# Nostrademous/dotaclient

Measured on AMD Instinct MI355X. Metric: PPO optimizer samples/sec (whole node) + actor steps/sec, 1v1-mid LSTM policy, higher is better.
Workload: dtype fp32

## Files before the change

### dotaclient_amd/ops/csrc/lstm_team.hip

```cpp
#include "common.h"
#include <cstdlib>

namespace {

using dca::bf16x8;
typedef int i32x4 __attribute__((ext_vector_type(4)));
typedef unsigned u32x2 __attribute__((ext_vector_type(2)));

constexpr int kT = 32;
constexpr int kMaxTeams = 8;
constexpr int kThreads = 256;
constexpr int kSc1 = 16;
constexpr int kPlain = 0;
constexpr unsigned kSpinLimit = 1u << 22;

struct TeamCtl {
  unsigned xcnt[16];
  unsigned state[kMaxTeams];
  unsigned chain[kMaxTeams];
  unsigned done[kMaxTeams];
  unsigned next_chain;
  unsigned abort;
  unsigned exits;
  unsigned epoch;
};
static_assert(sizeof(TeamCtl) <= 256, "TeamCtl must fit the 256-byte control tensor");

__device__ __forceinline__ unsigned xcc_id() { return __builtin_amdgcn_s_getreg((3 << 11) | 20) & 0xf; }
__device__ __forceinline__ unsigned ld_acq(const unsigned* p) {
  return __hip_atomic_load((__attribute__((address_space(1))) unsigned*)p, __ATOMIC_RELAXED, __HIP_MEMORY_SCOPE_AGENT);
}
__device__ __forceinline__ void st_rel(unsigned* p, unsigned v) {
  __hip_atomic_store((__attribute__((address_space(1))) unsigned*)p, v, __ATOMIC_RELAXED, __HIP_MEMORY_SCOPE_AGENT);
}
__device__ __forceinline__ unsigned add_agent(unsigned* p, unsigned v) {
  return __hip_atomic_fetch_add(p, v, __ATOMIC_RELAXED, __HIP_MEMORY_SCOPE_AGENT);
}
template <typename T>
__device__ __forceinline__ void gstore(T* p, T v) { *(__attribute__((address_space(1))) T*)p = v; }
__device__ __forceinline__ void lds_barrier() { asm volatile("s_waitcnt lgkmcnt(0)\n\ts_barrier" ::: "memory"); }

__device__ __forceinline__ void split_frag(const float* __restrict__ p, bf16x8& hi, bf16x8& lo) {
  const float4 a = *reinterpret_cast<const float4*>(p), b = *reinterpret_cast<const float4*>(p + 4);
  const float v[8] = {a.x, a.y, a.z, a.w, b.x, b.y, b.z, b.w};
#pragma unroll
  for (int j = 0; j < 8; ++j) {
    hi[j] = dca::f2bf(v[j]);
    lo[j] = dca::f2bf(v[j] - dca::bf2f(hi[j]));
  }
}

typedef float f32x2 __attribute__((ext_vector_type(2)));
template <int KSL>
__device__ __forceinline__ void pk_dot4(const float* wq, const float* x, float& o0, float& o1, float& o2, float& o3) {
  f32x2 a01e = {0.f, 0.f}, a01o = {0.f, 0.f}, a23e = {0.f, 0.f}, a23o = {0.f, 0.f};
#pragma unroll
  for (int j = 0; j < KSL; j += 4) {
    const float4 v = *reinterpret_cast<const float4*>(x + j);
    a01e = __builtin_elementwise_fma(f32x2{wq[j], wq[KSL + j]}, f32x2{v.x, v.x}, a01e);
    a23e = __builtin_elementwise_fma(f32x2{wq[2 * KSL + j], wq[3 * KSL + j]}, f32x2{v.x, v.x}, a23e);
    a01o = __builtin_elementwise_fma(f32x2{wq[j + 1], wq[KSL + j + 1]}, f32x2{v.y, v.y}, a01o);
    a23o = __builtin_elementwise_fma(f32x2{wq[2 * KSL + j + 1], wq[3 * KSL + j + 1]}, f32x2{v.y, v.y}, a23o);
    a01e = __builtin_elementwise_fma(f32x2{wq[j + 2], wq[KSL + j + 2]}, f32x2{v.z, v.z}, a01e);
    a23e = __builtin_elementwise_fma(f32x2{wq[2 * KSL + j + 2], wq[3 * KSL + j + 2]}, f32x2{v.z, v.z}, a23e);
    a01o = __builtin_elementwise_fma(f32x2{wq[j + 3], wq[KSL + j + 3]}, f32x2{v.w, v.w}, a01o);
    a23o = __builtin_elementwise_fma(f32x2{wq[2 * KSL + j + 3], wq[3 * KSL + j + 3]}, f32x2{v.w, v.w}, a23o);
  }
  const f32x2 a01 = a01e + a01o, a23 = a23e + a23o;
  o0 = a01.x; o1 = a01.y; o2 = a23.x; o3 = a23.y;
}
__device__ __forceinline__ float row_sum16(float v) {
  v += __int_as_float(__builtin_amdgcn_mov_dpp(__float_as_int(v), 0xB1, 0xF, 0xF, false));
  v += __int_as_float(__builtin_amdgcn_mov_dpp(__float_as_int(v), 0x4E, 0xF, 0xF, false));
  v += __int_as_float(__builtin_amdgcn_mov_dpp(__float_as_int(v), 0x141, 0xF, 0xF, false));
  v += __int_as_float(__builtin_amdgcn_mov_dpp(__float_as_int(v), 0x140, 0xF, 0xF, false));
  return v;
}

template <bool PREC>
__device__ __forceinline__ float sigm(float x) { return PREC ? 1.f / (1.f + expf(-x)) : dca::sigmoidf_(x); }
template <bool PREC>
__device__ __forceinline__ float tanh_(float x) { return PREC ? tanhf(x) : dca::tanhf_(x); }

__device__ __forceinline__ float row_sum32(float v) {
  v = row_sum16(v);
  return v + __int_as_float(__builtin_amdgcn_ds_swizzle(__float_as_int(v), 0x401F));
}

__device__ __forceinline__ __amdgpu_buffer_rsrc_t uniform_rsrc(const void* p, int bytes) {
  const unsigned long long a = (unsigned long long)p;
  const unsigned lo = __builtin_amdgcn_readfirstlane((unsigned)a);
  const unsigned hi = __builtin_amdgcn_readfirstlane((unsigned)(a >> 32));
  return __builtin_amdgcn_make_buffer_rsrc((void*)(((unsigned long long)hi << 32) | lo), (short)0,
                                           __builtin_amdgcn_readfirstlane(bytes), 0x00020000);
}

__device__ __forceinline__ bool spin_fail(unsigned& spins, unsigned long long& since, TeamCtl* ctl, unsigned* err,
                                          unsigned code, int knobs) {
  asm volatile("" ::: "memory");
  ++spins;
  if ((spins & 255u) == 0) {
    if (ld_acq(&ctl->abort) != 0) return true;
    const unsigned long long limit = ((knobs >> 15) & 1) ? 6000000000ull : 200000000ull;
    const unsigned long long now = __builtin_amdgcn_s_memrealtime();
    if (since == 0) {
      since = now;
    } else if (now - since > limit) {
      st_rel(err, code);
      st_rel(&ctl->abort, 1u);
      return true;
    }
  }
  if (spins > 32 && !((knobs >> 13) & 1)) __builtin_amdgcn_s_sleep(1);
  return false;
}

__device__ int join_team(TeamCtl* ctl, unsigned* err, int* sh, unsigned* sh_epoch, bool refuse = false) {
  if (threadIdx.x == 0) {
    *sh_epoch = ld_acq(&ctl->epoch);
    int res = -1;
    const unsigned x = xcc_id();
    if (x < kMaxTeams && !refuse) {
      const unsigned r = add_agent(&ctl->xcnt[x], 1u);
      if (r < (unsigned)kT) {
        res = (int)x * 64 + (int)r;
        unsigned spins = 0;
        if (r == 0) {
          bool ok = false;
          while (true) {
            if (ld_acq(&ctl->xcnt[x]) >= (unsigned)kT) { ok = true; break; }
            if (++spins > (1u << 16)) break;
            __builtin_amdgcn_s_sleep(2);
          }
          st_rel(&ctl->state[x], ok ? 1u : 2u);
          if (!ok) res = -1;
        } else {
          unsigned s;
          while ((s = ld_acq(&ctl->state[x])) == 0) {
            if (++spins > (1u << 18)) break;
            __builtin_amdgcn_s_sleep(2);
          }
          if (s != 1) res = -1;
        }
      }
    }
    *sh = res;
  }
  __syncthreads();
  return *sh;
}

__device__ int next_chain(TeamCtl* ctl, int team, int member, unsigned iter, int nch, int* sh) {
  if (threadIdx.x == 0) {
    int res = -1;
    unsigned spins = 0;
    if (member == 0) {
      while (ld_acq(&ctl->done[team]) < (unsigned)kT * iter) {
        if (ld_acq(&ctl->abort) || ++spins > (1u << 24)) { spins = ~0u; break; }
        __builtin_amdgcn_s_sleep(1);
      }
      unsigned c = spins == ~0u ? 0xffffu : add_agent(&ctl->next_chain, 1u);
      if (c > 0xffffu) c = 0xffffu;
      st_rel(&ctl->chain[team], ((iter + 1) << 16) | c);
      res = (c < (unsigned)nch) ? (int)c : -1;
    } else {
      unsigned v;
      while (((v = ld_acq(&ctl->chain[team])) >> 16) != iter + 1) {
        if (ld_acq(&ctl->abort) || ++spins > (1u << 24)) { v = 0xffffu; break; }
        __builtin_amdgcn_s_sleep(1);
      }
      const unsigned c = v & 0xffffu;
      res = (c < (unsigned)nch) ? (int)c : -1;
    }
    *sh = res;
  }
  __syncthreads();
  return *sh;
}

__device__ void team_exit(TeamCtl* ctl, unsigned* err, int nch) {
  __syncthreads();
  if (threadIdx.x == 0) {
    const unsigned e = add_agent(&ctl->exits, 1u);
    if (e == gridDim.x - 1) {
      if (ld_acq(&ctl->next_chain) < (unsigned)nch) st_rel(err, 3u);
      for (int i = 0; i < 16; ++i) st_rel(&ctl->xcnt[i], 0u);
      for (int i = 0; i < kMaxTeams; ++i) {
        st_rel(&ctl->state[i], 0u);
        st_rel(&ctl->chain[i], 0u);
        st_rel(&ctl->done[i], 0u);
      }
      st_rel(&ctl->next_chain, 0u);
      st_rel(&ctl->abort, 0u);
      st_rel(&ctl->exits, 0u);
      st_rel(&ctl->epoch, ld_acq(&ctl->epoch) + 1u);
    }
  }
}

__device__ __forceinline__ unsigned make_tagbase(unsigned epoch, unsigned iter) {
  return ((epoch & 0x7ffu) << 21) | (((iter + 1u) & 0x1fu) << 16);
}

template <int MT, int KS, bool F32, int VAR>
__device__ __forceinline__ void lstm_team_fwd_body(
    const float* __restrict__ xp4, const void* __restrict__ whh_, const float* __restrict__ h0,
    const float* __restrict__ c0, short* __restrict__ hs, float* __restrict__ hsf, float* __restrict__ cs,
    float* __restrict__ gates4, float* __restrict__ hn, float* __restrict__ cn, unsigned long long* xg_all,
    TeamCtl* ctl, unsigned* err, int Btot, int Bc, int nch, int S, int sb, int st, unsigned long long* trace,
    int knobs, const float* __restrict__ bias4, const unsigned char* __restrict__ rst) {
  constexpr int H = 128 * KS;
  constexpr int U = H / kT;
  constexpr int NTILE = U / 4;
  constexpr int KSTEP = H / 32;
  constexpr int HP = H + 8;
  constexpr int RB = MT * 16;
  constexpr int VV = VAR & 3;
  constexpr bool PREC = (VAR & 4) != 0;
  constexpr bool V1 = VV >= 1;
  constexpr int NT = VV == 2 ? 512 : kThreads;
  constexpr int LPU = VV == 2 ? 32 : 16;
  constexpr int UPW = 64 / LPU;
  constexpr int KSL = H / LPU;
  constexpr int R = V1 ? (1 << ((VAR >> 5) & 3)) : 1;
  constexpr int NR = V1 ? R : MT;
  static_assert(!V1 || (F32 && MT == 1), "V1 is the fp32 exact VALU variant");
  static_assert(VV != 2 || H == 512, "V2 maps 8 waves x 2 units onto the 16 units of H = 512");
  __shared__ short hl[V1 ? 1 : 2][V1 ? 1 : RB][V1 ? 1 : HP];
  __shared__ short hlo[F32 && !V1 ? 2 : 1][F32 && !V1 ? RB : 1][F32 && !V1 ? HP : 1];
  constexpr int SP = KSL + 4;
  constexpr int ROWF = LPU * SP;
  __shared__ __attribute__((aligned(16))) float hf[V1 ? 2 : 1][V1 ? R * ROWF : 4];
  __shared__ int sh_int;
  __shared__ unsigned sh_epoch;

  const int tid = threadIdx.x, wv = tid >> 6, lane = tid & 63;
  const int me = join_team(ctl, err, &sh_int, &sh_epoch, (knobs >> 11) & 1);
  const unsigned epoch = sh_epoch;
  if (me < 0) return;
  const int team = me >> 6, m = me & 63;
  const int j0 = m * U;
#define TSTAMP(ev)                                                                                        \
  if (trace && lane == 0 && wv < 4 && chain == 0 && t < 64)                                                \
    trace[(((size_t)m * 4 + wv) * 64 + t) * 8 + (ev)] = __builtin_amdgcn_s_memrealtime()
  constexpr int GPR = F32 ? H : H / 2;
  unsigned long long* xg = xg_all + (size_t)team * 2 * Bc * GPR;

  if constexpr (!V1)
    for (int i = tid; i < 2 * RB * HP; i += NT) (&hl[0][0][0])[i] = 0;
  if constexpr (F32 && !V1)
    for (int i = tid; i < 2 * RB * HP; i += NT) (&hlo[0][0][0])[i] = 0;

  const bool mfma_wave = VV == 2 || wv < NTILE;
  const int col = lane & 15, kg = lane >> 4;
  bf16x8 wf[V1 ? 1 : KSTEP];
  bf16x8 wfl[F32 && !V1 ? KSTEP : 1];
  float wq[V1 ? 4 * KSL : 1];
  if (mfma_wave) {
    const int row = (col & 3) * H + j0 + 4 * wv + (col >> 2);
    if constexpr (V1) {
#pragma unroll
      for (int g = 0; g < 4; ++g) {
        const float* wr = static_cast<const float*>(whh_) + (size_t)(g * H + j0 + UPW * wv + lane / LPU) * H +
                          (lane % LPU) * KSL;
#pragma unroll
        for (int j = 0; j < KSL; j += 4) {
          const float4 v = *reinterpret_cast<const float4*>(wr + j);
          wq[g * KSL + j] = v.x; wq[g * KSL + j + 1] = v.y; wq[g * KSL + j + 2] = v.z; wq[g * KSL + j + 3] = v.w;
        }
      }
    } else if constexpr (F32) {
      const float* whh = static_cast<const float*>(whh_);
#pragma unroll
      for (int ks = 0; ks < KSTEP; ++ks) split_frag(whh + (size_t)row * H + ks * 32 + 8 * kg, wf[ks], wfl[ks]);
    } else {
      const short* whh = static_cast<const short*>(whh_);
#pragma unroll
      for (int ks = 0; ks < KSTEP; ++ks)
        wf[ks] = *reinterpret_cast<const bf16x8*>(whh + (size_t)row * H + ks * 32 + 8 * kg);
    }
  }
  const int erow = V1 ? (lane % LPU) : 4 * kg + (col & 3);
  const int eunit = j0 + (V1 ? UPW * wv + lane / LPU : 4 * wv + (col >> 2));
  const dca::f32x4 bv = (bias4 && mfma_wave) ? *reinterpret_cast<const dca::f32x4*>(bias4 + eunit * 4)
                                             : dca::f32x4{0.f, 0.f, 0.f, 0.f};

  const int slice = V1 ? lane % LPU : 0;
  unsigned spins = 0;
  unsigned long long since = 0;
  for (unsigned iter = 0;; ++iter) {
    const int chain = next_chain(ctl, team, m, iter, nch, &sh_int);
    if (chain < 0) break;
    const int b0 = chain * Bc;
    const int B = min(Bc, Btot - b0);
    const unsigned tagbase = make_tagbase(epoch, iter);
    float creg[NR], hreg[NR];
#pragma unroll
    for (int i = 0; i < NR; ++i) {
      const int b = V1 ? i : i * 16 + erow;
      creg[i] = (mfma_wave && b < B) ? c0[(size_t)(b0 + b) * H + eunit] : 0.f;
      hreg[i] = 0.f;
    }
    bool dead = false;
    for (int t = 0; t < S; ++t) {
      const int par = t & 1;
      spins = 0;
      since = 0;
      TSTAMP(0);
      dca::f32x4 xv[NR];
      int rzb[NR];
      if (mfma_wave) {
#pragma unroll
        for (int i = 0; i < NR; ++i) {
          const int b = V1 ? i : i * 16 + erow;
          const size_t tx = ((knobs >> 10) & 1) ? 0 : (size_t)t;
          xv[i] = (b < B) ? *reinterpret_cast<const dca::f32x4*>(xp4 + (((size_t)(b0 + b) * sb + tx * st) * H + eunit) * 4)
                          : dca::f32x4{0.f, 0.f, 0.f, 0.f};
          rzb[i] = 0;
          if (rst != nullptr)
            rzb[i] = rst[(size_t)(b0 + (b < B ? b : 0)) * sb + (size_t)t * st];
        }
      }
      if (t == 0) {
        for (int i = tid; i < B * H; i += NT) {
          const int b = i / H, k = i % H;
          const float v = h0[(size_t)(b0 + b) * H + k];
          if constexpr (V1) {
            hf[par][b * ROWF + (k / KSL) * SP + k % KSL] = v;
          } else {
            hl[par][b][k] = dca::f2bf(v);
            if constexpr (F32) hlo[par][b][k] = dca::f2bf(v - dca::bf2f(dca::f2bf(v)));
          }
        }
      } else {
        const unsigned tag = tagbase | (unsigned)t;
        const __amdgpu_buffer_rsrc_t rs = uniform_rsrc(xg + (size_t)((t - 1) & 1) * Bc * GPR, Bc * GPR * 8);
        constexpr int CPR = F32 ? H / 2 : H / 4;
        constexpr int NL = ((V1 ? R : RB) * CPR + NT - 1) / NT;
        i32x4 g[NL];
        bool okc[NL];
#pragma unroll
        for (int i = 0; i < NL; ++i) okc[i] = tid + NT * i >= B * CPR;
        for (int i = 0; i < (knobs & 0xff); ++i) __builtin_amdgcn_s_sleep(1);
        if ((knobs >> 9) & 1) {
          while (!okc[0]) {
            g[0] = __builtin_amdgcn_raw_buffer_load_b128(rs, tid * 16, 0, kSc1);
            okc[0] = ((unsigned)g[0].y == tag) & ((unsigned)g[0].w == tag);
            if (__all(okc[0])) break;
            if (spin_fail(spins, since, ctl, err, 1u, knobs)) { dead = true; break; }
          }
        }
        while (!dead) {
#pragma unroll
          for (int i = 0; i < NL; ++i)
            if (!okc[i]) g[i] = __builtin_amdgcn_raw_buffer_load_b128(rs, (tid + NT * i) * 16, 0, kSc1);
          bool ok = true;
#pragma unroll
          for (int i = 0; i < NL; ++i) {
            okc[i] = okc[i] || (((unsigned)g[i].y == tag) & ((unsigned)g[i].w == tag));
            ok &= okc[i];
          }
          if (__all(ok)) break;
          if (spin_fail(spins, since, ctl, err, 1u, knobs)) { dead = true; break; }
        }
#pragma unroll
        for (int i = 0; i < NL; ++i) {
          const int ci = tid + NT * i;
          if (ci < B * CPR) {
            if constexpr (V1) {
              const int b = ci / CPR, k = 2 * (ci % CPR);
              *reinterpret_cast<float2*>(&hf[par][b * ROWF + (k / KSL) * SP + k % KSL]) =
                  make_float2(__int_as_float(g[i].x), __int_as_float(g[i].z));
            } else if constexpr (F32) {
              const int b = ci / CPR, k = (ci % CPR) * 2;
              const float x = __int_as_float(g[i].x), z = __int_as_float(g[i].z);
              const short xh = dca::f2bf(x), zh = dca::f2bf(z);
              *reinterpret_cast<unsigned*>(&hl[par][b][k]) = (unsigned)(unsigned short)xh | ((unsigned)(unsigned short)zh << 16);
              *reinterpret_cast<unsigned*>(&hlo[par][b][k]) =
                  (unsigned)(unsigned short)dca::f2bf(x - dca::bf2f(xh)) |
                  ((unsigned)(unsigned short)dca::f2bf(z - dca::bf2f(zh)) << 16);
            } else {
              const int b = ci / CPR, k = (ci % CPR) * 4;
              *reinterpret_cast<u32x2*>(&hl[par][b][k]) = u32x2{(unsigned)g[i].x, (unsigned)g[i].z};
            }
          }
        }
      }
      TSTAMP(1);
      if (dead) sh_int = -2;
      lds_barrier();
      if (sh_int == -2) break;
      TSTAMP(2);
      if constexpr (V1) {
       if (mfma_wave) {
        float g[R][4];
#pragma unroll
        for (int r = 0; r < R; ++r) {
          if (r < B) {
            pk_dot4<KSL>(wq, &hf[par][r * ROWF + slice * SP], g[r][0], g[r][1], g[r][2], g[r][3]);
#pragma unroll
            for (int q = 0; q < 4; ++q) g[r][q] = LPU == 32 ? row_sum32(g[r][q]) : row_sum16(g[r][q]);
          }
        }
        float act[R][4], cr[R], hr[R], hpub = 0.f;
#pragma unroll
        for (int r = 0; r < R; ++r) {
          cr[r] = hr[r] = 0.f;
          act[r][0] = act[r][1] = act[r][2] = act[r][3] = 0.f;
          if (r < B) {
            if (rzb[r]) { g[r][0] = 0.f; g[r][1] = 0.f; g[r][2] = 0.f; g[r][3] = 0.f; }
            const float pi = g[r][0] + (xv[r][0] + bv[0]), pf = g[r][1] + (xv[r][1] + bv[1]),
                        pg = g[r][2] + (xv[r][2] + bv[2]), po = g[r][3] + (xv[r][3] + bv[3]);
            const float ig = sigm<PREC>(pi), fg = sigm<PREC>(pf), gg = tanh_<PREC>(pg), og = sigm<PREC>(po);
            const float c = fg * (rzb[r] ? 0.f : creg[r]) + ig * gg;
            const float hv = og * tanh_<PREC>(c);
            creg[r] = c; hreg[r] = hv; cr[r] = c; hr[r] = hv;
            act[r][0] = ig; act[r][1] = fg; act[r][2] = gg; act[r][3] = og;
            if (slice == r) hpub = hv;
          }
        }
        TSTAMP(3);
        if (slice < B) {
          const u32x2 gv = {(unsigned)__float_as_int(hpub), tagbase | (unsigned)(t + 1)};
          const __amdgpu_buffer_rsrc_t ws = uniform_rsrc(xg + (size_t)par * Bc * GPR, Bc * GPR * 8);
          __builtin_amdgcn_raw_buffer_store_b64(gv, ws, (slice * H + eunit) * 8, 0, kPlain);
        }
        TSTAMP(4);
        const int orow = slice >> 1;
        if (orow < B && orow < R && !((knobs >> 8) & 1)) {
          float cv = 0.f, hv = 0.f;
          dca::f32x4 av = {0.f, 0.f, 0.f, 0.f};
#pragma unroll
          for (int r = 0; r < R; ++r)
            if (orow == r) { cv = cr[r]; hv = hr[r]; av = dca::f32x4{act[r][0], act[r][1], act[r][2], act[r][3]}; }
          const size_t o = ((size_t)(b0 + orow) * sb + (size_t)t * st) * H + eunit;
          gstore((slice & 1) ? hsf + o : cs + o, (slice & 1) ? hv : cv);
          if (!(slice & 1)) *reinterpret_cast<dca::f32x4*>(gates4 + o * 4) = av;
        }
        TSTAMP(5);
       }
      } else if (mfma_wave) {
#pragma unroll
        for (int mt = 0; mt < MT; ++mt) {
          if (mt * 16 >= B) break;
          float gq0 = 0.f, gq1 = 0.f, gq2 = 0.f, gq3 = 0.f;
          {
          dca::f32x4 acc = {0.f, 0.f, 0.f, 0.f};
          if constexpr (F32) {
            dca::f32x4 a1 = {0.f, 0.f, 0.f, 0.f}, a2 = {0.f, 0.f, 0.f, 0.f};
#pragma unroll
            for (int ks = 0; ks < KSTEP; ++ks) {
              const bf16x8 a = *reinterpret_cast<const bf16x8*>(&hl[par][mt * 16 + col][ks * 32 + 8 * kg]);
              const bf16x8 al = *reinterpret_cast<const bf16x8*>(&hlo[par][mt * 16 + col][ks * 32 + 8 * kg]);
              acc = __builtin_amdgcn_mfma_f32_16x16x32_bf16(a, wf[ks], acc, 0, 0, 0);
              a1 = __builtin_amdgcn_mfma_f32_16x16x32_bf16(al, wf[ks], a1, 0, 0, 0);
              a2 = __builtin_amdgcn_mfma_f32_16x16x32_bf16(a, wfl[ks], a2, 0, 0, 0);
            }
            acc += a1 + a2;
          } else {
#pragma unroll
            for (int ks = 0; ks < KSTEP; ++ks) {
              const bf16x8 a = *reinterpret_cast<const bf16x8*>(&hl[par][mt * 16 + col][ks * 32 + 8 * kg]);
              acc = __builtin_amdgcn_mfma_f32_16x16x32_bf16(a, wf[ks], acc, 0, 0, 0);
            }
          }
          const int q0 = col & 3;
#pragma unroll
          for (int j = 0; j < 4; ++j) {
            const int sel = (q0 - j) & 3;
            const float send = sel == 0 ? acc[0] : sel == 1 ? acc[1] : sel == 2 ? acc[2] : acc[3];
            const int qs = (q0 + j) & 3;
            float got = send;
            if (j == 1) got = __int_as_float(__builtin_amdgcn_mov_dpp(__float_as_int(send), 0x39, 0xF, 0xF, false));
            if (j == 2) got = __int_as_float(__builtin_amdgcn_mov_dpp(__float_as_int(send), 0x4E, 0xF, 0xF, false));
            if (j == 3) got = __int_as_float(__builtin_amdgcn_mov_dpp(__float_as_int(send), 0x93, 0xF, 0xF, false));
            gq0 = qs == 0 ? got : gq0;
            gq1 = qs == 1 ? got : gq1;
            gq2 = qs == 2 ? got : gq2;
            gq3 = qs == 3 ? got : gq3;
          }
          }
          const int b = mt * 16 + erow;
          if (rzb[mt]) { gq0 = 0.f; gq1 = 0.f; gq2 = 0.f; gq3 = 0.f; }
          const float pi = gq0 + (xv[mt][0] + bv[0]), pf = gq1 + (xv[mt][1] + bv[1]), pg = gq2 + (xv[mt][2] + bv[2]),
                      po = gq3 + (xv[mt][3] + bv[3]);
          const float ig = sigm<PREC>(pi), fg = sigm<PREC>(pf), gg = tanh_<PREC>(pg), og = sigm<PREC>(po);
          const float c = fg * (rzb[mt] ? 0.f : creg[mt]) + ig * gg;
          const float hv = og * tanh_<PREC>(c);
          if (b < B) { creg[mt] = c; hreg[mt] = hv; }
          TSTAMP(3);
          if constexpr (F32) {
            if (b < B) {
              const u32x2 gv = {(unsigned)__float_as_int(hv), tagbase | (unsigned)(t + 1)};
              const __amdgpu_buffer_rsrc_t ws = uniform_rsrc(xg + (size_t)par * Bc * GPR, Bc * GPR * 8);
              __builtin_amdgcn_raw_buffer_store_b64(gv, ws, (b * H + eunit) * 8, 0, kPlain);
            }
          } else {
            const float hnb = __int_as_float(__builtin_amdgcn_mov_dpp(__float_as_int(hv), 0x104, 0xF, 0xF, false));
            if (b < B && ((col >> 2) & 1) == 0) {
              const unsigned pl = (unsigned)(unsigned short)dca::f2bf(hv) | ((unsigned)(unsigned short)dca::f2bf(hnb) << 16);
              const u32x2 gv = {pl, tagbase | (unsigned)(t + 1)};
              const __amdgpu_buffer_rsrc_t ws = uniform_rsrc(xg + (size_t)par * Bc * GPR, Bc * GPR * 8);
              __builtin_amdgcn_raw_buffer_store_b64(gv, ws, (b * (H / 2) + (eunit >> 1)) * 8, 0, kPlain);
            }
          }
          TSTAMP(4);
          if (b < B && !((knobs >> 8) & 1)) {
            const size_t bt = (size_t)(b0 + b) * sb + (size_t)t * st;
            if (hs) hs[bt * H + eunit] = dca::f2bf(hv);
            if (hsf) hsf[bt * H + eunit] = hv;
            cs[bt * H + eunit] = c;
            *reinterpret_cast<dca::f32x4*>(gates4 + (bt * H + eunit) * 4) = dca::f32x4{ig, fg, gg, og};
          }
          TSTAMP(5);
        }
      }
    }
#undef TSTAMP
    if (sh_int == -2) return;
    if (mfma_wave) {
#pragma unroll
      for (int i = 0; i < NR; ++i) {
        const int b = V1 ? i : i * 16 + erow;
        if (b < B && (!V1 || slice == i)) {
          hn[(size_t)(b0 + b) * H + eunit] = hreg[i];
          cn[(size_t)(b0 + b) * H + eunit] = creg[i];
        }
      }
    }
    __syncthreads();
    if (tid == 0) add_agent(&ctl->done[team], 1u);
  }
}

template <int MT, int KS, bool F32, int VAR>
__device__ __forceinline__ void lstm_team_bwd_body(
    const float* __restrict__ dhs, const float* __restrict__ gates4, const float* __restrict__ cs,
    const float* __restrict__ c0, const float* __restrict__ dhn, const float* __restrict__ dcn,
    const void* __restrict__ whh_, float* __restrict__ dgates4, float* __restrict__ dh0, float* __restrict__ dc0,
    i32x4* xg_all, TeamCtl* ctl, unsigned* err, int Btot, int Bc, int nch, int S, int sb, int st,
    unsigned long long* trace, short* __restrict__ dg16, float* __restrict__ dbpart, int knobs,
    const unsigned char* __restrict__ rst) {
  constexpr int H = 128 * KS;
  constexpr int U = H / kT;
  constexpr int VV = VAR & 3;
  constexpr bool PREC = (VAR & 4) != 0;
  constexpr bool V1 = VV >= 1;
  constexpr int NWK = VV == 2 ? 8 : 4;
  constexpr int NT = 64 * NWK;
  constexpr int KW = 4 * H / NWK;
  constexpr int KSTEP = KW / 32;
  constexpr int RB = MT * 16;
  constexpr int GP = 4 * H + 8;
  constexpr int KSL = KW / 16;
  constexpr int R = V1 ? (1 << ((VAR >> 5) & 3)) : 1;
  constexpr int NPAIR = ((V1 ? R : RB) * U + NT - 1) / NT;
  static_assert(!V1 || (F32 && MT == 1), "V1 is the fp32 exact VALU variant");
  static_assert(VV != 2 || H == 512, "V2 is the H = 512 variant");
  __shared__ short dgl[V1 ? 1 : RB][V1 ? 1 : GP];
  __shared__ short dglo[F32 && !V1 ? RB : 1][F32 && !V1 ? GP : 1];
  constexpr int SP = KSL + 4;
  constexpr int DROW = (4 * H / KSL) * SP;
  __shared__ __attribute__((aligned(16))) float dgf[V1 ? R * DROW : 4];
  constexpr int RR = V1 ? R : RB;
  __shared__ float red[V1 ? 2 : 1][NWK][RR][16 + 1];
  __shared__ float dbs[RB * U * 4];
  __shared__ int sh_int;
  __shared__ unsigned sh_epoch;
  constexpr int kRstWords = 2048;
  __shared__ unsigned rbits[kRstWords];

  const int tid = threadIdx.x, wv = tid >> 6, lane = tid & 63;
  const int me = join_team(ctl, err, &sh_int, &sh_epoch);
  const unsigned epoch = sh_epoch;
  if (me < 0) return;
  const int team = me >> 6, m = me & 63;
  const int j0 = m * U;
  const int wpr = (S + 31) >> 5;
  constexpr int CPU_ = F32 ? 2 : 1;
  i32x4* xg = xg_all + (size_t)team * 2 * Bc * H * CPU_;
#define TSTAMPB(ev)                                                                                       \
  if (trace && lane == 0 && wv < 4 && chain == 0 && k < 64)                                               \
    trace[(((size_t)m * 4 + wv) * 64 + k) * 8 + (ev)] = __builtin_amdgcn_s_memrealtime()

  if constexpr (!V1)
    for (int i = tid; i < RB * GP; i += NT) (&dgl[0][0])[i] = 0;
  if constexpr (F32 && !V1)
    for (int i = tid; i < RB * GP; i += NT) (&dglo[0][0])[i] = 0;

  const int col = lane & 15, kg = lane >> 4;
  bf16x8 wf[V1 ? 1 : KSTEP];
  bf16x8 wfl[F32 && !V1 ? KSTEP : 1];
  float wq[V1 ? 4 * KSL : 1];
  if constexpr (V1) {
#pragma unroll
    for (int uu = 0; uu < 4; ++uu) {
      const int unit = 16 * (wv / NWK) + 4 * (lane >> 4) + uu;
#pragma unroll
      for (int j = 0; j < KSL; ++j) {
        const int gc = (wv % NWK) * KW + (lane & 15) * KSL + j;
        wq[uu * KSL + j] =
            (unit < U) ? static_cast<const float*>(whh_)[(size_t)((gc & 3) * H + (gc >> 2)) * H + j0 + unit] : 0.f;
      }
    }
  }
#pragma unroll
  for (int ks = 0; ks < (V1 ? 0 : KSTEP); ++ks) {
    bf16x8 v, vl;
#pragma unroll
    for (int j = 0; j < 8; ++j) {
      const int gc = wv * KW + ks * 32 + 8 * kg + j;
      const size_t wi = (size_t)((gc & 3) * H + (gc >> 2)) * H + j0 + col;
      if constexpr (F32) {
        const float w = (col < U) ? static_cast<const float*>(whh_)[wi] : 0.f;
        v[j] = dca::f2bf(w);
        vl[j] = dca::f2bf(w - dca::bf2f(v[j]));
      } else {
        v[j] = (col < U) ? static_cast<const short*>(whh_)[wi] : (short)0;
      }
    }
    wf[ks] = v;
    if constexpr (F32 && !V1) wfl[ks] = vl;
  }

  unsigned spins = 0;
  unsigned long long since = 0;
  for (unsigned iter = 0;; ++iter) {
    const int chain = next_chain(ctl, team, m, iter, nch, &sh_int);
    if (chain < 0) break;
    const int b0 = chain * Bc;
    const int B = min(Bc, Btot - b0);
    const unsigned tagbase = make_tagbase(epoch, iter);
    const bool rl = rst != nullptr && B * wpr <= kRstWords;
    if (rl) {
      for (int w = tid; w < B * wpr; w += NT) {
        const int b = w / wpr, tb = (w - b * wpr) * 32;
        const unsigned char* fr = rst + (size_t)(b0 + b) * sb;
        unsigned v = 0;
#pragma unroll
        for (int j = 0; j < 32; ++j)
          if (tb + j < S) v |= (fr[(size_t)(tb + j) * st] != 0 ? 1u : 0u) << j;
        rbits[w] = v;
      }
      lds_barrier();
    }
    float dcarry[NPAIR];
    dca::f32x4 dsum[NPAIR];
#pragma unroll
    for (int i = 0; i < NPAIR; ++i) dsum[i] = dca::f32x4{0.f, 0.f, 0.f, 0.f};
#pragma unroll
    for (int i = 0; i < NPAIR; ++i) {
      const int pi = tid + NT * i;
      dcarry[i] = (pi < B * U && dcn) ? dcn[(size_t)(b0 + pi / U) * H + j0 + pi % U] : 0.f;
    }
    bool dead = false;
    for (int k = 0; k <= S; ++k) {
      const int t = S - 1 - k;
      spins = 0;
      since = 0;
      TSTAMPB(0);
      dca::f32x4 gv[NPAIR];
      float cv[NPAIR], cpv[NPAIR], dv[NPAIR];
      bool rcur[NPAIR], rnext[NPAIR];
      if (t >= 0) {
#pragma unroll
        for (int i = 0; i < NPAIR; ++i) {
          const int pi = tid + NT * i;
          rcur[i] = rnext[i] = false;
          if (pi < B * U) {
            const int b = pi / U, u = pi % U;
            const size_t bt = (size_t)(b0 + b) * sb + (size_t)t * st;
            gv[i] = *reinterpret_cast<const dca::f32x4*>(gates4 + (bt * H + j0 + u) * 4);
            cv[i] = cs[bt * H + j0 + u];
            cpv[i] = t > 0 ? cs[(bt - st) * H + j0 + u] : c0[(size_t)(b0 + b) * H + j0 + u];
            dv[i] = dhs[bt * H + j0 + u];
            if (rl) {
              const unsigned* rw = rbits + b * wpr;
              rcur[i] = (rw[t >> 5] >> (t & 31)) & 1u;
              rnext[i] = t + 1 < S && ((rw[(t + 1) >> 5] >> ((t + 1) & 31)) & 1u);
            } else if (rst != nullptr) {
              rcur[i] = rst[bt] != 0;
              rnext[i] = t + 1 < S && rst[bt + st] != 0;
            }
          }
        }
      }
      if (k > 0) {
        const unsigned tag = tagbase | (unsigned)(t + 2);
        const __amdgpu_buffer_rsrc_t rs = uniform_rsrc(xg + (size_t)((t + 1) & 1) * Bc * H * CPU_, Bc * H * CPU_ * 16);
        constexpr int RG = F32 ? 4 : 8;
        constexpr int NL = RG * H * CPU_ / NT;
        if constexpr (V1) {
          constexpr int CW = KW / 128;
          constexpr int NLW = R * CW;
          static_assert(KW % 128 == 0, "a wave's K part is whole rounds of 64 chunks");
          const int cw0 = (wv % NWK) * (KW / 2) + lane;
          i32x4 g[NLW];
          bool okc[NLW];
#pragma unroll
          for (int i = 0; i < NLW; ++i) okc[i] = i / CW >= B;
          while (true) {
#pragma unroll
            for (int i = 0; i < NLW; ++i)
              if (!okc[i])
                g[i] = __builtin_amdgcn_raw_buffer_load_b128(rs, ((i / CW) * H * CPU_ + cw0 + 64 * (i % CW)) * 16, 0, kSc1);
            bool ok = true;
#pragma unroll
            for (int i = 0; i < NLW; ++i) {
              okc[i] = okc[i] || (((unsigned)g[i].y == tag) & ((unsigned)g[i].w == tag));
              ok &= okc[i];
            }
            if (__all(ok)) break;
            if (spin_fail(spins, since, ctl, err, 2u, knobs)) { dead = true; break; }
          }
#pragma unroll
          for (int i = 0; i < NLW; ++i) {
            if (i / CW < B) {
              const int r = cw0 + 64 * (i % CW), gc = 4 * (r >> 1) + 2 * (r & 1);
              *reinterpret_cast<float2*>(&dgf[(i / CW) * DROW + (gc / KSL) * SP + gc % KSL]) =
                  make_float2(__int_as_float(g[i].x), __int_as_float(g[i].z));
            }
          }
        } else {
          for (int g0 = 0; g0 < B && !dead; g0 += RG) {
            const int nck = min(RG, B - g0) * H * CPU_;
            i32x4 g[NL];
            bool okc[NL];
#pragma unroll
            for (int i = 0; i < NL; ++i) okc[i] = tid + NT * i >= nck;
            while (true) {
#pragma unroll
              for (int i = 0; i < NL; ++i)
                if (!okc[i]) g[i] = __builtin_amdgcn_raw_buffer_load_b128(rs, (g0 * H * CPU_ + tid + NT * i) * 16, 0, kSc1);
              bool ok = true;
#pragma unroll
              for (int i = 0; i < NL; ++i) {
                okc[i] = okc[i] || (((unsigned)g[i].y == tag) & ((unsigned)g[i].w == tag));
                ok &= okc[i];
              }
              if (__all(ok)) break;
              if (spin_fail(spins, since, ctl, err, 2u, knobs)) { dead = true; break; }
            }
#pragma unroll
            for (int i = 0; i < NL; ++i) {
              const int ci = tid + NT * i;
              if (ci < nck) {
                if constexpr (F32) {
                  const int b = g0 + ci / (2 * H), r = ci % (2 * H), gc = 4 * (r >> 1) + 2 * (r & 1);
                  const float x = __int_as_float(g[i].x), z = __int_as_float(g[i].z);
                  const short xh = dca::f2bf(x), zh = dca::f2bf(z);
                  *reinterpret_cast<unsigned*>(&dgl[b][gc]) = (unsigned)(unsigned short)xh | ((unsigned)(unsigned short)zh << 16);
                  *reinterpret_cast<unsigned*>(&dglo[b][gc]) =
                      (unsigned)(unsigned short)dca::f2bf(x - dca::bf2f(xh)) |
                      ((unsigned)(unsigned short)dca::f2bf(z - dca::bf2f(zh)) << 16);
                } else {
                  const int b = g0 + ci / H, j = ci % H;
                  *reinterpret_cast<u32x2*>(&dgl[b][4 * j]) = u32x2{(unsigned)g[i].x, (unsigned)g[i].z};
                }
              }
            }
          }
        }
      }
      TSTAMPB(1);
      if constexpr (V1) {
        asm volatile("s_waitcnt lgkmcnt(0)" ::: "memory");
      } else {
        if (dead) sh_int = -2;
        lds_barrier();
        if (sh_int == -2) break;
        TSTAMPB(2);
      }
      const int rp = V1 ? (k & 1) : 0;
      if (V1 && k > 0) {
       if (!dead) {
        const int wk = wv % NWK;
        const int u0 = 16 * (wv / NWK) + 4 * (lane >> 4);
#pragma unroll
        for (int r = 0; r < R; ++r) {
          if (r >= B) break;
          float o0, o1, o2, o3;
          const float* x = &dgf[r * DROW + (wk * 16 + (lane & 15)) * SP];
          pk_dot4<KSL>(wq, x, o0, o1, o2, o3);
          o0 = row_sum16(o0);
          o1 = row_sum16(o1);
          o2 = row_sum16(o2);
          o3 = row_sum16(o3);
          if ((lane & 15) == 0 && u0 < U) {
            red[rp][wk][r][u0] = o0;
            red[rp][wk][r][u0 + 1] = o1;
            red[rp][wk][r][u0 + 2] = o2;
            red[rp][wk][r][u0 + 3] = o3;
          }
        }
       }
      } else if (k > 0) {
#pragma unroll
        for (int mt = 0; mt < MT; ++mt) {
          if (mt * 16 >= B) break;
          dca::f32x4 acc = {0.f, 0.f, 0.f, 0.f};
          if constexpr (F32) {
            dca::f32x4 a1 = {0.f, 0.f, 0.f, 0.f}, a2 = {0.f, 0.f, 0.f, 0.f};
#pragma unroll
            for (int ks = 0; ks < KSTEP; ++ks) {
              const bf16x8 a = *reinterpret_cast<const bf16x8*>(&dgl[mt * 16 + col][wv * KW + ks * 32 + 8 * kg]);
              const bf16x8 al = *reinterpret_cast<const bf16x8*>(&dglo[mt * 16 + col][wv * KW + ks * 32 + 8 * kg]);
              acc = __builtin_amdgcn_mfma_f32_16x16x32_bf16(a, wf[ks], acc, 0, 0, 0);
              a1 = __builtin_amdgcn_mfma_f32_16x16x32_bf16(al, wf[ks], a1, 0, 0, 0);
              a2 = __builtin_amdgcn_mfma_f32_16x16x32_bf16(a, wfl[ks], a2, 0, 0, 0);
            }
            acc += a1 + a2;
          } else {
#pragma unroll
            for (int ks = 0; ks < KSTEP; ++ks) {
              const bf16x8 a = *reinterpret_cast<const bf16x8*>(&dgl[mt * 16 + col][wv * KW + ks * 32 + 8 * kg]);
              acc = __builtin_amdgcn_mfma_f32_16x16x32_bf16(a, wf[ks], acc, 0, 0, 0);
            }
          }
#pragma unroll
          for (int r = 0; r < 4; ++r) red[0][wv][mt * 16 + kg * 4 + r][col] = acc[r];
        }
      }
      TSTAMPB(3);
      if (V1 && dead) sh_int = -2;
      lds_barrier();
      if (V1 && sh_int == -2) break;
      TSTAMPB(4);
      if (t < 0) {
        for (int i = tid; i < B * U; i += NT) {
          const int b = i / U, u = i % U;
          float acc = 0.f;
#pragma unroll
          for (int w = 0; w < NWK; ++w) acc += red[rp][w][b][u];
          dh0[(size_t)(b0 + b) * H + j0 + u] = (rst != nullptr && rst[(size_t)(b0 + b) * sb] != 0) ? 0.f : acc;
        }
        break;
      }
      const __amdgpu_buffer_rsrc_t ws = uniform_rsrc(xg + (size_t)(t & 1) * Bc * H * CPU_, Bc * H * CPU_ * 16);
      const int tg = (int)(tagbase | (unsigned)(t + 1));
#pragma unroll
      for (int i = 0; i < NPAIR; ++i) {
        const int pi = tid + NT * i;
        if (pi < B * U) {
          const int b = pi / U, u = pi % U;
          float rec = 0.f;
          if (k == 0) {
            rec = dhn ? dhn[(size_t)(b0 + b) * H + j0 + u] : 0.f;
          } else if (!rnext[i]) {
#pragma unroll
            for (int w = 0; w < NWK; ++w) rec += red[rp][w][b][u];
          }
          const float ig = gv[i][0], fg = gv[i][1], gg = gv[i][2], og = gv[i][3];
          const float dht = dv[i] + rec;
          const float tc = tanh_<PREC>(cv[i]);
          const float dc = dcarry[i] + dht * og * (1.f - tc * tc);
          const float d_i = dc * gg * ig * (1.f - ig);
          const float d_f = rcur[i] ? 0.f : dc * cpv[i] * fg * (1.f - fg);
          const float d_g = dc * ig * (1.f - gg * gg);
          const float d_o = dht * tc * og * (1.f - og);
          dcarry[i] = rcur[i] ? 0.f : dc * fg;
          const size_t bt = (size_t)(b0 + b) * sb + (size_t)t * st;
          if constexpr (F32) {
            const int o = (b * H + j0 + u) * 2 * 16;
            __builtin_amdgcn_raw_buffer_store_b128(i32x4{__float_as_int(d_i), tg, __float_as_int(d_f), tg}, ws, o, 0,
                                                   kPlain);
            __builtin_amdgcn_raw_buffer_store_b128(i32x4{__float_as_int(d_g), tg, __float_as_int(d_o), tg}, ws, o + 16,
                                                   0, kPlain);
            *reinterpret_cast<dca::f32x4*>(dgates4 + (bt * H + j0 + u) * 4) = dca::f32x4{d_i, d_f, d_g, d_o};
          } else {
            const unsigned p01 = (unsigned)(unsigned short)dca::f2bf(d_i) | ((unsigned)(unsigned short)dca::f2bf(d_f) << 16);
            const unsigned p23 = (unsigned)(unsigned short)dca::f2bf(d_g) | ((unsigned)(unsigned short)dca::f2bf(d_o) << 16);
            __builtin_amdgcn_raw_buffer_store_b128(i32x4{(int)p01, tg, (int)p23, tg}, ws, (b * H + j0 + u) * 16, 0, kPlain);
            if (dg16) *reinterpret_cast<u32x2*>(dg16 + (bt * H + j0 + u) * 4) = u32x2{p01, p23};
            else *reinterpret_cast<dca::f32x4*>(dgates4 + (bt * H + j0 + u) * 4) = dca::f32x4{d_i, d_f, d_g, d_o};
          }
          dsum[i] += dca::f32x4{d_i, d_f, d_g, d_o};
          if (t == 0) dc0[(size_t)(b0 + b) * H + j0 + u] = dcarry[i];
        }
      }
      TSTAMPB(6);
    }
    if (sh_int == -2) return;
    if (dbpart) {
#pragma unroll
      for (int i = 0; i < NPAIR; ++i) {
        const int pi = tid + NT * i;
        if (pi < B * U) *reinterpret_cast<dca::f32x4*>(&dbs[pi * 4]) = dsum[i];
      }
      __syncthreads();
      for (int o = tid; o < U * 4; o += NT) {
        float acc = 0.f;
        for (int b = 0; b < B; ++b) acc += dbs[b * U * 4 + o];
        dbpart[(size_t)chain * 4 * H + (o & 3) * H + j0 + (o >> 2)] = acc;
      }
    }
    __syncthreads();
    if (tid == 0) add_agent(&ctl->done[team], 1u);
  }
#undef TSTAMPB
}

inline int team_threads(int var) { return (var & 3) == 2 ? 512 : kThreads; }

template <int MT, int KS, bool F32, int VAR>
__global__ __launch_bounds__((VAR & 3) == 2 ? 512 : kThreads, 1) void lstm_team_fwd_kernel(
    const float* __restrict__ xp4, const void* __restrict__ whh, const float* __restrict__ h0,
    const float* __restrict__ c0, short* __restrict__ hs, float* __restrict__ hsf, float* __restrict__ cs,
    float* __restrict__ gates4, float* __restrict__ hn, float* __restrict__ cn, unsigned long long* xg_all,
    TeamCtl* ctl, unsigned* err, int Btot, int Bc, int nch, int S, int sb, int st, unsigned long long* trace,
    int knobs, const float* __restrict__ bias4, const unsigned char* __restrict__ rst) {
  __builtin_amdgcn_s_setprio(3);
  lstm_team_fwd_body<MT, KS, F32, VAR>(xp4, whh, h0, c0, hs, hsf, cs, gates4, hn, cn, xg_all, ctl, err, Btot, Bc, nch, S, sb,
                             st, trace, knobs, bias4, rst);
  team_exit(ctl, err, nch);
}

template <int MT, int KS, bool F32, int VAR>
__global__ __launch_bounds__((VAR & 3) == 2 ? 512 : kThreads, 1) void lstm_team_bwd_kernel(
    const float* __restrict__ dhs, const float* __restrict__ gates4, const float* __restrict__ cs,
    const float* __restrict__ c0, const float* __restrict__ dhn, const float* __restrict__ dcn,
    const void* __restrict__ whh, float* __restrict__ dgates4, float* __restrict__ dh0, float* __restrict__ dc0,
    i32x4* xg_all, TeamCtl* ctl, unsigned* err, int Btot, int Bc, int nch, int S, int sb, int st,
    unsigned long long* trace, short* __restrict__ dg16, float* __restrict__ dbpart, int knobs,
    const unsigned char* __restrict__ rst) {
  __builtin_amdgcn_s_setprio(3);
  lstm_team_bwd_body<MT, KS, F32, VAR>(dhs, gates4, cs, c0, dhn, dcn, whh, dgates4, dh0, dc0, xg_all, ctl, err, Btot, Bc, nch,
                             S, sb, st, trace, dg16, dbpart, knobs, rst);
  team_exit(ctl, err, nch);
}

inline int team_knobs() {
  const char* e = getenv("DCA_TEAM_KNOBS");
  const char* f = getenv("DCA_TEAM_FAIL");
  const char* p = getenv("DCA_TEAM_PATIENT");
  return (e ? atoi(e) : 0) | ((f && f[0] == '1') ? (1 << 11) : 0) | ((p && p[0] == '1') ? (1 << 15) : 0);
}

inline void plan(int B, int& nch, int& Bc, int& MT, int f32 = 0) {
  nch = B <= kMaxTeams * 32 ? (B < kMaxTeams ? B : kMaxTeams) : (B + 31) / 32;
  if (f32 && (B + nch - 1) / nch > 16) nch = (B + 15) / 16;
  Bc = (B + nch - 1) / nch;
  MT = Bc <= 16 ? 1 : 2;
}

}

#define DCA_TEAM_DISPATCH(MT_, KS_, F32_, V1_, ...)                                                        \
  switch (((V1_) << 12) | ((F32_) << 8) | ((MT_) << 4) | (KS_)) {                                          \
    case 0x0011: return __VA_ARGS__(1, 1, false, 0); case 0x0012: return __VA_ARGS__(1, 2, false, 0); \
    case 0x0014: return __VA_ARGS__(1, 4, false, 0); case 0x0021: return __VA_ARGS__(2, 1, false, 0); \
    case 0x0022: return __VA_ARGS__(2, 2, false, 0); case 0x0024: return __VA_ARGS__(2, 4, false, 0); \
    case 0x0111: return __VA_ARGS__(1, 1, true, 0);  case 0x0112: return __VA_ARGS__(1, 2, true, 0);  \
    case 0x0114: return __VA_ARGS__(1, 4, true, 0);                                                      \
    case 0x1111: return __VA_ARGS__(1, 1, true, 1);      case 0x1112: return __VA_ARGS__(1, 2, true, 1);      \
    case 0x1114: return __VA_ARGS__(1, 4, true, 1);      case 0x2114: return __VA_ARGS__(1, 4, true, 2);      \
    case 0x5111: return __VA_ARGS__(1, 1, true, 5);      case 0x5112: return __VA_ARGS__(1, 2, true, 5);      \
    case 0x5114: return __VA_ARGS__(1, 4, true, 5);      case 0x6114: return __VA_ARGS__(1, 4, true, 6);      \
    case 0x21111: return __VA_ARGS__(1, 1, true, 33);    case 0x21112: return __VA_ARGS__(1, 2, true, 33);   \
    case 0x21114: return __VA_ARGS__(1, 4, true, 33);    case 0x22114: return __VA_ARGS__(1, 4, true, 34);   \
    case 0x41111: return __VA_ARGS__(1, 1, true, 65);    case 0x41112: return __VA_ARGS__(1, 2, true, 65);   \
    case 0x41114: return __VA_ARGS__(1, 4, true, 65);    case 0x42114: return __VA_ARGS__(1, 4, true, 66);   \
    default: return hipErrorInvalidValue;                                                                    \
  }

inline int use_v1(int f32, int Bc, int H, int backward, int precise) {
  if (!(f32 && Bc <= 4)) return 0;
  const int rows = Bc == 1 ? 0 : (Bc == 2 ? 32 : 64);
  return ((H == 512 && backward) ? 2 : 1) | (precise ? 4 : 0) | rows;
}

extern "C" size_t dca_lstm_team_ctl_bytes() { return 256; }

extern "C" int dca_lstm_team_chains(int B, int f32) {
  int nch, Bc, MT;
  plan(B, nch, Bc, MT, f32);
  return nch;
}

extern "C" size_t dca_lstm_team_workspace(int B, int H, int backward, int f32) {
  int nch, Bc, MT;
  plan(B, nch, Bc, MT, f32);
  if (!backward) return (size_t)kMaxTeams * 2 * Bc * (f32 ? H : H / 2) * 8;
  return (size_t)kMaxTeams * 2 * Bc * H * (f32 ? 2 : 1) * 16;
}

extern "C" hipError_t dca_lstm_team_fwd(const float* xp4, const void* whh, const float* h0, const float* c0,
                                        short* hs, float* hsf, float* cs, float* gates4, float* hn, float* cn,
                                        void* ctl_mem, void* ws, size_t ws_bytes, unsigned* err, int B, int S, int H,
                                        int time_major, hipStream_t stream, unsigned long long* trace,
                                        const float* bias4, int f32, int precise, const unsigned char* rst) {
  if (B < 1 || S < 1 || S >= 65535 || (H != 128 && H != 256 && H != 512)) return hipErrorInvalidValue;
  if (ws_bytes < dca_lstm_team_workspace(B, H, 0, f32) || ctl_mem == nullptr) return hipErrorInvalidValue;
  if (f32 && hsf == nullptr) return hipErrorInvalidValue;
  if (!f32 && hs == nullptr) return hipErrorInvalidValue;
  int nch, Bc, MT;
  plan(B, nch, Bc, MT, f32);
  const int sb = time_major ? 1 : S, st = time_major ? B : 1;
  TeamCtl* ctl = reinterpret_cast<TeamCtl*>(ctl_mem);
  unsigned long long* xg = reinterpret_cast<unsigned long long*>(ws);
  const int KS = H / 128;
#define DCA_F(mt, ks, f, v)                                                                                     \
  (lstm_team_fwd_kernel<mt, ks, f, v><<<kMaxTeams * kT, team_threads(v), 0, stream>>>(xp4, whh, h0, c0, hs, hsf, cs, gates4, \
                                                                          hn, cn, xg, ctl, err, B, Bc, nch, S, sb, \
                                                                          st, trace, team_knobs(), bias4, rst),    \
   hipGetLastError())
  DCA_TEAM_DISPATCH(MT, KS, f32 ? 1 : 0, use_v1(f32, Bc, H, 0, precise), DCA_F)
#undef DCA_F
}

extern "C" hipError_t dca_lstm_team_bwd(const float* dhs, const float* gates4, const float* cs, const float* c0,
                                        const float* dhn, const float* dcn, const void* whh, float* dgates4,
                                        float* dh0, float* dc0, void* ctl_mem, void* ws, size_t ws_bytes,
                                        unsigned* err, int B, int S, int H, int time_major, hipStream_t stream,
                                        unsigned long long* trace, short* dg16, float* dbpart, int f32, int precise,
                                        const unsigned char* rst) {
  if (B < 1 || S < 1 || S >= 65534 || (H != 128 && H != 256 && H != 512)) return hipErrorInvalidValue;
  if (dgates4 == nullptr && dg16 == nullptr) return hipErrorInvalidValue;
  if (f32 && dgates4 == nullptr) return hipErrorInvalidValue;
  if (ws_bytes < dca_lstm_team_workspace(B, H, 1, f32) || ctl_mem == nullptr) return hipErrorInvalidValue;
  int nch, Bc, MT;
  plan(B, nch, Bc, MT, f32);
  const int sb = time_major ? 1 : S, st = time_major ? B : 1;
  TeamCtl* ctl = reinterpret_cast<TeamCtl*>(ctl_mem);
  i32x4* xb = reinterpret_cast<i32x4*>(ws);
  const int KS = H / 128;
#define DCA_B(mt, ks, f, v)                                                                                        \
  (lstm_team_bwd_kernel<mt, ks, f, v><<<kMaxTeams * kT, team_threads(v), 0, stream>>>(dhs, gates4, cs, c0, dhn, dcn, whh,      \
                                                                          dgates4, dh0, dc0, xb, ctl, err, B, Bc,  \
                                                                          nch, S, sb, st, trace, dg16, dbpart,      \
                                                                          team_knobs(), rst),                      \
   hipGetLastError())
  DCA_TEAM_DISPATCH(MT, KS, f32 ? 1 : 0, use_v1(f32, Bc, H, 1, precise), DCA_B)
#undef DCA_B
}
```

Measured before the change: 2.169 million.

## Exchange dh instead of gate grads in V1 LSTM backward, recompute gates per consumer

For the fp32 V1 backward variant with a single row and small per-wave unit slices, each team block now publishes only dh plus a tag (an 8-byte record) to the exchange buffer instead of four gate gradients (two 16-byte records). Each consumer lane recomputes the gate gradients for the units it needs from preloaded activations, cell state and the reset bits, writing them to LDS. The owning block also writes dgates and dc0 and keeps the bias sums. Activations for the next step are prefetched after the wait. This cuts cross-block exchange traffic and polling bytes on the serial recurrence, at the cost of redundant gate-gradient arithmetic in every block and some extra register pressure.

```diff
diff --git a/dotaclient_amd/ops/csrc/lstm_team.hip b/dotaclient_amd/ops/csrc/lstm_team.hip
--- a/dotaclient_amd/ops/csrc/lstm_team.hip
+++ b/dotaclient_amd/ops/csrc/lstm_team.hip
@@ -13,6 +13,7 @@
 constexpr int kSc1 = 16;
 constexpr int kPlain = 0;
 constexpr unsigned kSpinLimit = 1u << 22;
+constexpr bool kActsAhead = true;
 
 struct TeamCtl {
   unsigned xcnt[16];
@@ -533,6 +534,25 @@
   }
 }
 
+__device__ __forceinline__ dca::f32x4 gate_grads(const dca::f32x4 gv, float tc, float cpv, float dht, bool rcur,
+                                                 float& dcarry, dca::f32x4& sum) {
+#pragma clang fp contract(off)
+  const float ig = gv[0], fg = gv[1], gg = gv[2], og = gv[3];
+  const float dc = __builtin_fmaf(dht * og, __builtin_fmaf(-tc, tc, 1.f), dcarry);
+  const float d_i = dc * gg * ig * (1.f - ig);
+  const float d_f = rcur ? 0.f : dc * cpv * fg * (1.f - fg);
+  const float qg = 1.f - gg * gg, qo = 1.f - og;
+  const float pg = dc * ig, po = dht * tc * og;
+  const float d_g = pg * qg;
+  const float d_o = po * qo;
+  dcarry = rcur ? 0.f : dc * fg;
+  sum[0] += d_i;
+  sum[1] += d_f;
+  sum[2] = __builtin_fmaf(pg, qg, sum[2]);
+  sum[3] = __builtin_fmaf(po, qo, sum[3]);
+  return dca::f32x4{d_i, d_f, d_g, d_o};
+}
+
 template <int MT, int KS, bool F32, int VAR>
 __device__ __forceinline__ void lstm_team_bwd_body(
     const float* __restrict__ dhs, const float* __restrict__ gates4, const float* __restrict__ cs,
@@ -555,6 +575,8 @@
   constexpr int KSL = KW / 16;
   constexpr int R = V1 ? (1 << ((VAR >> 5) & 3)) : 1;
   constexpr int NPAIR = ((V1 ? R : RB) * U + NT - 1) / NT;
+  constexpr int UW = KW / 4;
+  constexpr bool HO = V1 && UW <= 64 && R == 1;
   static_assert(!V1 || (F32 && MT == 1), "V1 is the fp32 exact VALU variant");
   static_assert(VV != 2 || H == 512, "V2 is the H = 512 variant");
   __shared__ short dgl[V1 ? 1 : RB][V1 ? 1 : GP];
@@ -653,6 +675,36 @@
       const int pi = tid + NT * i;
       dcarry[i] = (pi < B * U && dcn) ? dcn[(size_t)(b0 + pi / U) * H + j0 + pi % U] : 0.f;
     }
+    constexpr int RH = HO ? R : 1;
+    const int cu = (wv % NWK) * UW + lane;
+    const bool hasu = HO && lane < UW;
+    const bool mine = hasu && cu >= j0 && cu < j0 + U;
+    dca::f32x4 cg[RH], csum[RH];
+    float ccv[RH], ccp[RH], ctc[RH], cdc[RH];
+    bool crc[RH];
+    auto load_acts = [&](int s) {
+#pragma unroll
+      for (int r = 0; r < RH; ++r) {
+        if (r < B && hasu) {
+          const size_t bt = (size_t)(b0 + r) * sb + (size_t)s * st;
+          cg[r] = *reinterpret_cast<const dca::f32x4*>(gates4 + (bt * H + cu) * 4);
+          ccp[r] = s > 0 ? cs[(bt - st) * H + cu] : c0[(size_t)(b0 + r) * H + cu];
+        }
+      }
+    };
+    if constexpr (HO) {
+#pragma unroll
+      for (int r = 0; r < RH; ++r) {
+        const bool on = r < B && hasu;
+        csum[r] = dca::f32x4{0.f, 0.f, 0.f, 0.f};
+        cg[r] = dca::f32x4{0.f, 0.f, 0.f, 0.f};
+        ccp[r] = ctc[r] = 0.f;
+        crc[r] = false;
+        cdc[r] = (on && dcn) ? dcn[(size_t)(b0 + r) * H + cu] : 0.f;
+        ccv[r] = on ? cs[((size_t)(b0 + r) * sb + (size_t)(S - 1) * st) * H + cu] : 0.f;
+        asm volatile("" ::"v"(ccv[r]));
+      }
+    }
     bool dead = false;
     for (int k = 0; k <= S; ++k) {
       const int t = S - 1 - k;
@@ -660,9 +712,37 @@
       since = 0;
       TSTAMPB(0);
       dca::f32x4 gv[NPAIR];
-      float cv[NPAIR], cpv[NPAIR], dv[NPAIR];
+      float cv[NPAIR], cpv[NPAIR], dv[NPAIR], dvl[NPAIR];
       bool rcur[NPAIR], rnext[NPAIR];
-      if (t >= 0) {
+      if constexpr (HO) {
+        if (t >= 0) {
+#pragma unroll
+          for (int i = 0; i < NPAIR; ++i) {
+            const int pi = tid + NT * i;
+            rnext[i] = false;
+            if (pi < B * U) {
+              const int b = pi / U, u = pi % U;
+              const size_t bt = (size_t)(b0 + b) * sb + (size_t)t * st;
+              dv[i] = dhs[bt * H + j0 + u];
+              if (rl) rnext[i] = t + 1 < S && ((rbits[b * wpr + ((t + 1) >> 5)] >> ((t + 1) & 31)) & 1u);
+              else if (rst != nullptr) rnext[i] = t + 1 < S && rst[bt + st] != 0;
+            }
+          }
+        }
+        if (k > 0) {
+          if constexpr (!kActsAhead) load_acts(t + 1);
+#pragma unroll
+          for (int r = 0; r < RH; ++r) {
+            if (r < B && hasu) {
+              ctc[r] = tanh_<PREC>(ccv[r]);
+              if (rl) crc[r] = (rbits[r * wpr + ((t + 1) >> 5)] >> ((t + 1) & 31)) & 1u;
+              else if (rst != nullptr) crc[r] = rst[(size_t)(b0 + r) * sb + (size_t)(t + 1) * st] != 0;
+            }
+          }
+        } else if constexpr (kActsAhead) {
+          load_acts(t);
+        }
+      } else if (t >= 0) {
 #pragma unroll
         for (int i = 0; i < NPAIR; ++i) {
           const int pi = tid + NT * i;
@@ -690,7 +770,52 @@
         const __amdgpu_buffer_rsrc_t rs = uniform_rsrc(xg + (size_t)((t + 1) & 1) * Bc * H * CPU_, Bc * H * CPU_ * 16);
         constexpr int RG = F32 ? 4 : 8;
         constexpr int NL = RG * H * CPU_ / NT;
-        if constexpr (V1) {
+        if constexpr (HO) {
+          const __amdgpu_buffer_rsrc_t rh =
+              uniform_rsrc(reinterpret_cast<const char*>(xg) + (size_t)((t + 1) & 1) * Bc * H * 8, Bc * H * 8);
+          u32x2 g[RH];
+          bool okc[RH];
+#pragma unroll
+          for (int r = 0; r < RH; ++r) {
+            okc[r] = r >= B || !hasu;
+            g[r] = u32x2{0u, 0u};
+          }
+          while (true) {
+#pragma unroll
+            for (int r = 0; r < RH; ++r)
+              if (!okc[r]) g[r] = __builtin_amdgcn_raw_buffer_load_b64(rh, (r * H + cu) * 8, 0, kSc1);
+            bool ok = true;
+#pragma unroll
+            for (int r = 0; r < RH; ++r) {
+              okc[r] = okc[r] || g[r].y == tag;
+              ok &= okc[r];
+            }
+            if (__all(ok)) break;
+            if (spin_fail(spins, since, ctl, err, 2u, knobs)) { dead = true; break; }
+          }
+#pragma unroll
+          for (int i = 0; i < NPAIR; ++i) asm volatile("v_mov_b32 %0, %1" : "=v"(dvl[i]) : "v"(dv[i]));
+          if (!dead) {
+#pragma unroll
+            for (int r = 0; r < RH; ++r) {
+              if (r < B && hasu) {
+                const dca::f32x4 d =
+                    gate_grads(cg[r], ctc[r], ccp[r], __uint_as_float(g[r].x), crc[r], cdc[r], csum[r]);
+                constexpr int gpl = KSL / 4;
+                *reinterpret_cast<dca::f32x4*>(&dgf[r * DROW + (cu / gpl) * SP + (cu % gpl) * 4]) = d;
+                if (mine) {
+                  const size_t bt = (size_t)(b0 + r) * sb + (size_t)(t + 1) * st;
+                  *reinterpret_cast<dca::f32x4*>(dgates4 + (bt * H + cu) * 4) = d;
+                  if (t + 1 == 0) dc0[(size_t)(b0 + r) * H + cu] = cdc[r];
+                }
+                ccv[r] = ccp[r];
+              }
+            }
+            if constexpr (kActsAhead)
+              if (t >= 0) load_acts(t);
+          }
+          TSTAMPB(5);
+        } else if constexpr (V1) {
           constexpr int CW = KW / 128;
           constexpr int NLW = R * CW;
           static_assert(KW % 128 == 0, "a wave's K part is whole rounds of 64 chunks");
@@ -838,6 +963,28 @@
       }
       const __amdgpu_buffer_rsrc_t ws = uniform_rsrc(xg + (size_t)(t & 1) * Bc * H * CPU_, Bc * H * CPU_ * 16);
       const int tg = (int)(tagbase | (unsigned)(t + 1));
+      if constexpr (HO) {
+        const __amdgpu_buffer_rsrc_t wh =
+            uniform_rsrc(reinterpret_cast<const char*>(xg) + (size_t)(t & 1) * Bc * H * 8, Bc * H * 8);
+#pragma unroll
+        for (int i = 0; i < NPAIR; ++i) {
+          const int pi = tid + NT * i;
+          if (pi < B * U) {
+            const int b = pi / U, u = pi % U;
+            float rec = 0.f;
+            if (k == 0) {
+              rec = dhn ? dhn[(size_t)(b0 + b) * H + j0 + u] : 0.f;
+              asm volatile("v_mov_b32 %0, %2\n\tv_mov_b32 %1, %3" : "=&v"(dvl[i]), "=v"(rec) : "v"(dv[i]), "v"(rec));
+            } else if (!rnext[i]) {
+#pragma unroll
+              for (int w = 0; w < NWK; ++w) rec += red[rp][w][b][u];
+            }
+            const float dht = dvl[i] + rec;
+            __builtin_amdgcn_raw_buffer_store_b64(u32x2{__float_as_uint(dht), (unsigned)tg}, wh, (b * H + j0 + u) * 8, 0,
+                                                  kPlain);
+          }
+        }
+      } else {
 #pragma unroll
       for (int i = 0; i < NPAIR; ++i) {
         const int pi = tid + NT * i;
@@ -878,14 +1025,21 @@
           if (t == 0) dc0[(size_t)(b0 + b) * H + j0 + u] = dcarry[i];
         }
       }
+      }
       TSTAMPB(6);
     }
     if (sh_int == -2) return;
     if (dbpart) {
-#pragma unroll
-      for (int i = 0; i < NPAIR; ++i) {
-        const int pi = tid + NT * i;
-        if (pi < B * U) *reinterpret_cast<dca::f32x4*>(&dbs[pi * 4]) = dsum[i];
+      if constexpr (HO) {
+#pragma unroll
+        for (int r = 0; r < RH; ++r)
+          if (r < B && mine) *reinterpret_cast<dca::f32x4*>(&dbs[(r * U + cu - j0) * 4]) = csum[r];
+      } else {
+#pragma unroll
+        for (int i = 0; i < NPAIR; ++i) {
+          const int pi = tid + NT * i;
+          if (pi < B * U) *reinterpret_cast<dca::f32x4*>(&dbs[pi * 4]) = dsum[i];
+        }
       }
       __syncthreads();
       for (int o = tid; o < U * 4; o += NT) {
```

New measurement: 2.221 million, median of 6. 1.02x the previous value.
